# CognitiveAISystems/pogema

Hardware: AMD Instinct MI355X
Metric: agent-steps/sec (whole node), 64-agent 64x64 grid, batch=8192 envs (higher is better)
Workload: dtype u32

## Files before the change

include/pogema_amd.h:

```cpp
#ifndef POGEMA_AMD_H
#define POGEMA_AMD_H

#include <stddef.h>
#include <stdint.h>

#ifdef __cplusplus
extern "C" {
#endif

#define PGX_ABI_VERSION 6

#define PGX_OK 0
#define PGX_E_INVALID (-1)
#define PGX_E_HIP (-2)
#define PGX_E_NOMEM (-3)
#define PGX_E_STATE (-4)
#define PGX_E_PLACEMENT (-5)

#define PGX_COLLISION_PRIORITY 0
#define PGX_COLLISION_BLOCK_BOTH 1
#define PGX_COLLISION_SOFT 2

#define PGX_ON_TARGET_FINISH 0
#define PGX_ON_TARGET_RESTART 1
// ... 51 lines not shown
int pgx_abi_version(void);
const char* pgx_last_error(void);

int pgx_create(const pgx_config* cfg, int device, pgx_env** out);
int pgx_destroy(pgx_env* env);
int pgx_check_config(const pgx_config* cfg);

int64_t pgx_obs_elems(const pgx_env* env);
int64_t pgx_agent_elems(const pgx_env* env);

int pgx_reset_from_state(pgx_env* env, const uint8_t* obstacles, const int32_t* agent_xy,
                         const int32_t* target_xy, void* stream);

int pgx_reset_random(pgx_env* env, float density, uint64_t seed, const uint8_t* shared_map,
                     const uint8_t* env_mask, int32_t max_retries, void* stream);

int pgx_regenerate(pgx_env* env, const uint8_t* env_mask, float density, uint64_t seed, const uint8_t* shared_map,
                   int32_t max_retries, void* obs, void* stream);
int64_t pgx_regenerate_failures(pgx_env* env, void* stream);

int pgx_set_map_pool(pgx_env* env, const uint8_t* maps, int32_t num_maps, int32_t* capacity_out, void* stream);
int pgx_reset_pool(pgx_env* env, uint64_t seed, const uint8_t* env_mask, int32_t max_retries, void* stream);
int pgx_regenerate_pool(pgx_env* env, const uint8_t* env_mask, uint64_t seed, int32_t max_retries, void* obs,
                        void* stream);
int pgx_get_map_index(pgx_env* env, int32_t* map_index, void* stream);

int pgx_get_map(pgx_env* env, uint8_t* obstacles, void* stream);

int pgx_step(pgx_env* env, const void* actions, int action_dtype, void* obs, float* rewards,
             uint8_t* terminated, uint8_t* truncated, uint8_t* is_active, void* stream);

int pgx_step_held(pgx_env* env, const void* actions, int action_dtype, void* obs, uint8_t* held, int32_t refresh,
                  float* rewards, uint8_t* terminated, uint8_t* truncated, uint8_t* is_active, void* stream);
int pgx_held_available(const pgx_env* env);

int pgx_xcd_shares(pgx_env* env, int32_t* shares);
int pgx_xcd_tune(pgx_env* env, void* obs, void* obs_alt, int32_t rounds, float* us_equal, float* us_tuned, void* stream);

typedef struct pgx_geometry {
    int32_t lanes_per_env;
    int32_t waves;
    int32_t envs_per_wave;
    int32_t multi_wave;
    int32_t p16;
    int32_t stagger;
    int32_t store_policy;
    int32_t state_stores;
    int32_t grid;
    int32_t lds_bytes;
    int32_t for_rollout;
    int32_t xcd_aware;
} pgx_geometry;
int pgx_get_geometry(const pgx_env* env, int32_t for_rollout, pgx_geometry* out);

typedef struct pgx_rollout_io {
    const void* actions;
    void* obs;
    float* rewards;
    uint8_t* terminated;
    uint8_t* truncated;
    uint8_t* is_active;
    uint8_t* episode_done;
    float* metrics;
    int32_t action_dtype;
    int32_t obs_slots;
    int64_t obs_slot_stride;
// ... 141 lines not shown
```

pogema_amd/_lib.py:

```python
from __future__ import annotations

import ctypes as C
import os

_HERE = os.path.dirname(os.path.abspath(__file__))
LIB_PATH = os.environ.get("PGX_LIB") or os.path.join(_HERE, "libpogema_amd.so")

PGX_ABI_VERSION = 6

COLLISION_SYSTEMS = {"priority": 0, "block_both": 1, "soft": 2}
ON_TARGET = {"finish": 0, "restart": 1, "nothing": 2}
ACTION_DTYPES = {"int8": 0, "int32": 1, "int64": 2}
SOFT_VERTEX_RULES = {"lowest_index": 0, "all_stay": 1}
SOFT_OCCUPANCY = {"index_order": 0, "exact": 1}
COOP_REWARDS = {"all_solved": 0, "per_agent": 1}
BAD_ACTIONS = {"noop": 0, "flag": 1}
LIFELONG_RNGS = {"build": 0, "numpy": 1}
def _obs_dtypes():
    import torch
    return {torch.float32: 0, torch.uint8: 1, torch.bfloat16: 2, torch.float16: 3}


def obs_elem_bytes(dtype) -> int:
    import torch
# ... 9 lines not shown
    def __contains__(self, k):
        self._fill()
        return dict.__contains__(self, k)

    def __getitem__(self, k):
        self._fill()
        return dict.__getitem__(self, k)


OBS_DTYPES = _LazyObsDtypes()
METRIC_NAMES = ("ISR", "CSR", "ep_length", "SoC", "makespan", "avg_throughput")
MAX_OBS_RADIUS, MAX_AGENTS, MAX_SIDE = 15, 1024, 1024
MAX_NEIGHBOURS = 32
DIRECTIONS_FORMATS = {"float32": 0, "uint8": 1, "bits": 2}
SHIELD_TIE_BREAKS = {None: 0, "distance": 1}
MAX_PLAN_HORIZON = 256
PLAN_FIXED_PRIORITY = 1
OUTCOMES = ("STAY", "MOVED", "OBSTACLE", "SWAP", "OCCUPIED", "FOLLOW", "CONTESTED")
NUM_OUTCOMES = len(OUTCOMES)
POLICY_CHANNELS = {"obstacles": 0, "agents": 1, "target": 2, "other_goals": 3, "up": 4, "down": 5, "left": 6, "right": 7}
NUM_CHANNELS = len(POLICY_CHANNELS)
COPY_NO_CACHE = 1
DEFAULT_POLICY_CHANNELS = ("obstacles", "agents", "target", "up", "down", "left", "right")
GLOBAL_CHANNELS = {"obstacles": 0, "agents": 1, "targets": 2, "agent_ids": 3, "target_ids": 4}
NUM_GLOBAL_CHANNELS = len(GLOBAL_CHANNELS)
DEFAULT_GLOBAL_CHANNELS = ("obstacles", "agents", "targets")
GLOBAL_ID_CHANNELS = ("agent_ids", "target_ids")
GLOBAL_ID_MAX = {1: 255, 2: 256}
GLOBAL_BAND_CELLS = 8192


EXPORTED_SYMBOLS = (
    "pgx_abi_version", "pgx_last_error", "pgx_create", "pgx_check_config", "pgx_destroy", "pgx_obs_elems", "pgx_agent_elems",
    "pgx_reset_from_state", "pgx_reset_random", "pgx_regenerate", "pgx_regenerate_failures", "pgx_get_map", "pgx_step", "pgx_step_held", "pgx_held_available", "pgx_observe", "pgx_set_metrics_buffers", "pgx_get_state", "pgx_generate", "pgx_place_agents",
    "pgx_snapshot_bytes", "pgx_save_snapshot", "pgx_load_snapshot", "pgx_time_observe", "pgx_bad_action_count",
    "pgx_buffers_create", "pgx_buffers_ptr", "pgx_buffers_get_info", "pgx_buffers_destroy", "pgx_set_targets",
    "pgx_np_streams", "pgx_np_streams_host", "pgx_np_generate", "pgx_np_generate_host", "pgx_rollout", "pgx_buffers_stride", "pgx_buffers_drop", "pgx_xcd_shares", "pgx_xcd_tune", "pgx_buffers_create_at", "pgx_time_observe_pair", "pgx_buffers_va_reserved", "pgx_get_geometry",
    "pgx_expert_actions", "pgx_set_map_pool", "pgx_reset_pool", "pgx_regenerate_pool", "pgx_get_map_index",
    "pgx_cost_to_go", "pgx_cost_to_go_bytes", "pgx_cost_to_go_builds", "pgx_visible_agents", "pgx_pibt_actions",
    "pgx_goal_directions", "pgx_shield_actions", "pgx_pibt_plan", "pgx_move_outcomes",
    "pgx_policy_input", "pgx_copy_envs", "pgx_global_state", "pgx_global_state_check",
)


class PgxError(RuntimeError):
    def __init__(self, code: int, message: str):
        super().__init__(f"pogema_amd engine error {code}: {message}")
        self.code = code


class PgxBuffersInfo(C.Structure):
    _fields_ = [("bytes", C.c_int64), ("count", C.c_int32), ("spread", C.c_int32), ("candidates", C.c_int32),
                ("reserved0", C.c_int32), ("same_zone_us", C.c_float), ("final_us", C.c_float), ("spacer_gib", C.c_double),
                ("buffer_gbs", C.c_float), ("reserved1", C.c_float)]


class PgxGeometry(C.Structure):
    _fields_ = [(n, C.c_int32) for n in ("lanes_per_env", "waves", "envs_per_wave", "multi_wave", "p16", "stagger",
                                          "store_policy", "state_stores", "grid", "lds_bytes", "for_rollout", "xcd_aware")]


class PgxRolloutIO(C.Structure):
    _fields_ = [("actions", C.c_void_p), ("obs", C.c_void_p), ("rewards", C.c_void_p), ("terminated", C.c_void_p),
                ("truncated", C.c_void_p), ("is_active", C.c_void_p), ("episode_done", C.c_void_p), ("metrics", C.c_void_p),
                ("action_dtype", C.c_int32), ("obs_slots", C.c_int32), ("obs_slot_stride", C.c_int64),
                ("policy_seed", C.c_uint64), ("policy_step0", C.c_int64), ("actions_out", C.c_void_p)]

# ... 95 lines not shown
    lib.pgx_move_outcomes.argtypes = [vp, vp, i32, i32, vp, vp, vp, vp, vp]
    lib.pgx_move_outcomes.restype = C.c_int
    lib.pgx_policy_input.argtypes = [vp, C.POINTER(i32), i32, i32, vp, vp]
    lib.pgx_policy_input.restype = C.c_int
    lib.pgx_global_state.argtypes = [vp, C.POINTER(i32), i32, i32, vp, vp]
    lib.pgx_global_state.restype = C.c_int
    lib.pgx_global_state_check.argtypes = [i32, C.POINTER(i32), i32, i32, vp]
    lib.pgx_global_state_check.restype = C.c_int
    lib.pgx_copy_envs.argtypes = [vp, vp, vp, i32, i32, vp]
    lib.pgx_copy_envs.restype = C.c_int
    lib.pgx_set_map_pool.argtypes = [vp, vp, i32, vp, vp]
    lib.pgx_set_map_pool.restype = C.c_int
    lib.pgx_reset_pool.argtypes = [vp, u64, vp, i32, vp]
    lib.pgx_reset_pool.restype = C.c_int
    lib.pgx_regenerate_pool.argtypes = [vp, vp, u64, i32, vp, vp]
    lib.pgx_regenerate_pool.restype = C.c_int
    lib.pgx_get_map_index.argtypes = [vp, vp, vp]
    lib.pgx_get_map_index.restype = C.c_int
    lib.pgx_set_targets.argtypes = [vp, vp, vp, vp]
    lib.pgx_set_targets.restype = C.c_int
    lib.pgx_bad_action_count.argtypes = [vp, vp]
    lib.pgx_bad_action_count.restype = i64
    lib.pgx_time_observe.argtypes = [vp, vp, i32, C.POINTER(C.c_float), vp]
    lib.pgx_time_observe.restype = C.c_int
    lib.pgx_time_observe_pair.argtypes = [vp, vp, vp, i32, C.POINTER(C.c_float), vp]
    lib.pgx_time_observe_pair.restype = C.c_int
    lib.pgx_snapshot_bytes.argtypes = [vp]
    lib.pgx_snapshot_bytes.restype = i64
    lib.pgx_save_snapshot.argtypes = [vp, vp, vp]
    lib.pgx_load_snapshot.argtypes = [vp, vp, vp]
    lib.pgx_save_snapshot.restype = lib.pgx_load_snapshot.restype = C.c_int
    lib.pgx_step.argtypes = [vp, vp, C.c_int, vp, vp, vp, vp, vp, vp]
    lib.pgx_step_held.argtypes = [vp, vp, C.c_int, vp, vp, i32, vp, vp, vp, vp, vp]
    lib.pgx_held_available.argtypes = [vp]
    lib.pgx_step_held.restype = lib.pgx_held_available.restype = C.c_int
    lib.pgx_observe.argtypes = [vp, vp, vp]
    lib.pgx_set_metrics_buffers.argtypes = [vp, vp, vp]
    lib.pgx_get_state.argtypes = [vp, vp, vp, vp, vp, vp, vp]
    lib.pgx_generate.argtypes = [i32, i32, i32, i32, f32, u64, i64, i32, i32, vp, vp, vp]
    lib.pgx_place_agents.argtypes = [i32, i32, i32, i32, u64, i64, i32, i32, vp, i32, vp, vp]
    for name in ("pgx_create", "pgx_destroy", "pgx_reset_from_state", "pgx_reset_random", "pgx_regenerate", "pgx_get_map",
                 "pgx_step", "pgx_observe", "pgx_set_metrics_buffers", "pgx_set_metrics_buffers",
                 "pgx_get_state", "pgx_generate", "pgx_place_agents"):
        getattr(lib, name).restype = C.c_int
    if lib.pgx_abi_version() != PGX_ABI_VERSION:
        raise ImportError(f"{LIB_PATH}: ABI version {lib.pgx_abi_version()} != expected {PGX_ABI_VERSION}; rebuild")
    _lib = lib
    return lib


def check(status: int) -> None:
    if status != 0:
        msg = load().pgx_last_error()
        raise PgxError(status, msg.decode("utf-8", "replace") if msg else "unknown error")
```

pogema_amd/buffers.py:

```python
from __future__ import annotations

import atexit
import collections
import contextlib
import ctypes as C
import os
import threading

import numpy as np
import torch

from . import _lib

_TYPESTR = {torch.float32: "<f4", torch.uint8: "|u1", torch.float16: "<f2", torch.bfloat16: "<f2"}


class _Owner:

    def __init__(self, lib, handle):
        self._lib, self._handle = lib, handle

    def __del__(self):
        try:
            if self._handle is not None and self._handle.value:
# ... 303 lines not shown
    _HOOK = hook
    return hook


_UNSET = object()
_HOOK = _UNSET


class RecyclingOutputs:

    @staticmethod
    def available() -> bool:
        return storage_count_hook() is not None

    def __init__(self, obs_tensors, batch: int, agents: int, zone_ptrs=()):
        if not self.available():
            raise RuntimeError("torch._C._storage_Use_Count is missing or changed its meaning in this torch build")
        self._count = storage_count_hook()
        self._zone_ptrs = frozenset(int(p) for p in zone_ptrs)
        dev = obs_tensors[0].device
        n = batch * agents
        self._sets = []
        for obs in obs_tensors:
            block = torch.empty(n * 7 + 16, dtype=torch.uint8, device=dev)
            members = (obs, block[:4 * n].view(torch.float32).view(batch, agents),
                       block[4 * n:5 * n].view(torch.bool).view(batch, agents),
                       block[5 * n:6 * n].view(torch.bool).view(batch, agents),
                       block[6 * n:7 * n].view(torch.bool).view(batch, agents))
            storages = (obs.untyped_storage(), block.untyped_storage())
            self._sets.append((members, storages, tuple(st._cdata for st in storages)))
        del obs, block, members, storages
        self._idle = [tuple(self._count(c) for c in cdata) for _, _, cdata in self._sets]
        self._held = [torch.full((batch, agents), 255, dtype=torch.uint8, device=dev) for _ in self._sets]
        self._vouched = [None] * len(self._sets)
        self._next = 0
        self.taken = 0
        self.misses = 0

    def __len__(self):
        return len(self._sets)

    def obs_pointers(self):
        return [members[0].data_ptr() for members, _, _ in self._sets]

    def _is_idle(self, i: int) -> bool:
        cdata, idle = self._sets[i][2], self._idle[i]
        return self._count(cdata[0]) == idle[0] and self._count(cdata[1]) == idle[1]

    def free_sets(self) -> int:
        return sum(self._is_idle(i) for i in range(len(self._sets)))

    def retire(self):
        idle = [i for i in range(len(self._sets)) if self._is_idle(i)]
        out = [self._sets[i][0][0] for i in idle if self._sets[i][0][0].data_ptr() in self._zone_ptrs]
        for i in reversed(idle):
            del self._sets[i]
            del self._idle[i]
            del self._held[i]
            del self._vouched[i]
        self._next = 0
        return out

    def _take_index(self):
        n = len(self._sets)
        for k in range(n):
            i = (self._next + k) % n
            if self._is_idle(i):
                self._next = (i + 1) % n
                self.taken += 1
                return i
        self.misses += 1
        return None

    def _hand_out(self, i: int, with_obs: bool):
        m = self._sets[i][0]
        return (m[0].detach() if with_obs else None, m[1].detach(), m[2].detach(), m[3].detach(), m[4].detach())

    @staticmethod
    def _version(t):
        try:
            return t._version
        except Exception:
            return None

    def take(self, with_obs: bool = True):
        i = self._take_index()
        if i is None:
            return None
        if with_obs:
            self._vouched[i] = None
        return self._hand_out(i, with_obs)

    def take_for_step(self, with_obs: bool = True):
        i = self._take_index()
        if i is None:
            return None
        trusted = False
        if with_obs:
            v = self._vouched[i]
            trusted = v is not None and self._version(self._sets[i][0][0]) == v
            self._vouched[i] = None
        return self._hand_out(i, with_obs), self._held[i], trusted, i

    def vouch(self, i: int):
        self._vouched[i] = self._version(self._sets[i][0][0])
```

pogema_amd/csrc/pgx_api.cpp:

```cpp
#include "../../include/pogema_amd.h"

#include <hip/hip_runtime.h>

#include <algorithm>
#include <cstdarg>
#include <cstdio>
#include <cstdlib>
#include <cstring>
#include <new>
#include <string>
#include <vector>

#include "pgx_internal.h"

namespace {
thread_local std::string g_err;
}

namespace pgx {
int fail_msg(int code, const char* fmt, ...) {
    char buf[512];
    va_list ap;
    va_start(ap, fmt);
    vsnprintf(buf, sizeof buf, fmt, ap);
// ... 881 lines not shown
int pgx_get_map(pgx_env* e, uint8_t* obstacles, void* stream) {
    if (!e || !obstacles) return fail_msg(PGX_E_INVALID, "pgx_get_map: null argument");
    DeviceGuard guard;
    if (const int rc = enter(guard, e, "pgx_get_map", true)) return rc;
    PGX_HIP(hipMemcpyAsync(obstacles, e->map_u8, (size_t)e->cfg.batch * e->cfg.height * e->cfg.width,
                           hipMemcpyDeviceToDevice, (hipStream_t)stream));
    return PGX_OK;
}

int pgx_step(pgx_env* e, const void* actions, int action_dtype, void* obs, float* rewards, uint8_t* terminated,
             uint8_t* truncated, uint8_t* is_active, void* stream) {
    if (!e || !actions || !rewards || !terminated || !truncated) return fail_msg(PGX_E_INVALID, "pgx_step: null argument");
    if (const int rc = check_action_dtype("pgx_step", action_dtype)) return rc;
    DeviceGuard guard;
    if (const int rc = enter(guard, e, "pgx_step", true)) return rc;
    pgx::StepParams p = step_params(e, e->geo);
    p.mode = pgx::MODE_STEP;
    p.action_dtype = action_dtype;
    p.actions = actions;
    p.obs = static_cast<float*>(obs);
    p.rewards = rewards;
    p.terminated = terminated;
    p.truncated = truncated;
    p.act_out = is_active;
    PGX_HIP(pgx::launch_step(p, e->geo, (hipStream_t)stream));
    return PGX_OK;
}

int pgx_held_available(const pgx_env* e) {
    if (!e) return 0;
    return pgx::held_available(e->geo, e->cfg.num_agents, e->W, obs_elem_bytes(e->cfg.obs_dtype)) ? 1 : 0;
}

int pgx_step_held(pgx_env* e, const void* actions, int action_dtype, void* obs, uint8_t* held, int32_t refresh, float* rewards,
                  uint8_t* terminated, uint8_t* truncated, uint8_t* is_active, void* stream) {
    if (!e || !obs || !held || !pgx_held_available(e))
        return pgx_step(e, actions, action_dtype, obs, rewards, terminated, truncated, is_active, stream);
    if (!actions || !rewards || !terminated || !truncated) return fail_msg(PGX_E_INVALID, "pgx_step_held: null argument");
    if (const int rc = check_action_dtype("pgx_step_held", action_dtype)) return rc;
    DeviceGuard guard;
    if (const int rc = enter(guard, e, "pgx_step_held", true)) return rc;
    pgx::StepParams p = step_params(e, e->geo);
    p.mode = pgx::MODE_STEP;
    p.action_dtype = action_dtype;
    p.actions = actions;
    p.obs = static_cast<float*>(obs);
    p.rewards = rewards;
    p.terminated = terminated;
    p.truncated = truncated;
    p.act_out = is_active;
    PGX_HIP(pgx::launch_step_held(p, e->geo, held, refresh != 0, (hipStream_t)stream));
    return PGX_OK;
}

int pgx_rollout(pgx_env* e, int32_t steps, const pgx_rollout_io* io, void* stream) {
    if (!e || !io || !io->rewards || !io->terminated || !io->truncated)
        return fail_msg(PGX_E_INVALID, "pgx_rollout: null argument");
    if (io->policy_step0 < 0 || io->policy_step0 > ((int64_t)1 << 40))
        return fail_msg(PGX_E_INVALID, "pgx_rollout: policy_step0 outside 0..2^40");
    if (steps < 1) return fail_msg(PGX_E_INVALID, "pgx_rollout: steps must be >= 1, got %d", steps);
    if (const int rc = check_action_dtype("pgx_rollout", io->action_dtype)) return rc;
    if (io->obs && io->obs_slots < 1) return fail_msg(PGX_E_INVALID, "pgx_rollout: obs given but obs_slots = %d", io->obs_slots);
    DeviceGuard guard;
    if (const int rc = enter(guard, e, "pgx_rollout", true)) return rc;
    pgx::StepParams p = step_params(e, e->geo_roll);
    p.mode = pgx::MODE_STEP;
    p.action_dtype = io->action_dtype;
    p.actions = io->actions;
    p.obs = static_cast<float*>(io->obs);
    p.rewards = io->rewards;
    p.terminated = io->terminated;
    p.truncated = io->truncated;
    p.act_out = io->is_active;
    p.metrics_out = io->metrics;
    p.episode_done = io->episode_done;
    const int64_t agents = (int64_t)e->cfg.batch * e->cfg.num_agents;
    const int64_t W = 2 * e->cfg.obs_radius + 1;
    static const int64_t action_bytes[3] = {1, 4, 8};
    pgx::RolloutParams rp;
    rp.steps = steps;
    rp.obs_slots = io->obs ? io->obs_slots : 1;
    rp.resident_bitmap = e->geo_roll.resident_bitmap ? 1 : 0;
    rp.reserved0 = 0;
    rp.actions_stride = agents * action_bytes[io->action_dtype];
    rp.agents_stride = agents;
// ... 553 lines not shown
```

pogema_amd/csrc/pgx_internal.h:

```cpp
#pragma once
#include <hip/hip_runtime.h>
#include <stddef.h>
#include <stdint.h>

namespace pgx {

int fail_msg(int code, const char* fmt, ...);

#define PGX_HIP(call)                                                                                                      \
    do {                                                                                                                   \
        const hipError_t e__ = (call);                                                                                     \
        if (e__ != hipSuccess)                                                                                             \
            return pgx::fail_msg(PGX_E_HIP, "%s failed: %s (%s:%d)", #call, hipGetErrorString(e__), __FILE__, __LINE__); \
    } while (0)

struct DeviceGuard {
    int prev = -1;
    bool changed = false;
    hipError_t err = hipSuccess;
    DeviceGuard() = default;
    explicit DeviceGuard(int dev) { (void)select(dev); }
    DeviceGuard(const DeviceGuard&) = delete;
    DeviceGuard& operator=(const DeviceGuard&) = delete;
    hipError_t select(int dev) {
// ... 79 lines not shown
    int32_t xcd_base[8];
    uint32_t flags;
    uint64_t seed;
    int64_t env_index_base;
    const uint32_t* obst;
    uint32_t* pos;
    uint32_t* tgt;
    uint8_t* active;
    int32_t* elapsed;
    const uint32_t* pos0;
    const uint32_t* tgt0;
    const uint32_t* comp_begin;
    const uint32_t* comp_len;
    const uint32_t* comp_cells;
    uint32_t* tcount;
    NpGen* np_state;
    const NpGen* np_state0;
    int4* macc;
    float* metrics_out;
    uint8_t* episode_done;
    uint32_t* bad_count;
    const void* actions;
    float* obs;
    float* rewards;
    uint8_t* terminated;
    uint8_t* truncated;
    uint8_t* act_out;
    const uint8_t* only;
    unsigned long long* dbg;
};

struct HeldParams {
    uint8_t* held;
    int32_t refresh;
    int32_t lds_word;
    int32_t words;
};

struct RolloutParams {
    int32_t steps;
    int32_t obs_slots;
    int32_t resident_bitmap;
    int32_t reserved0;
    int64_t actions_stride;
    int64_t agents_stride;
    int64_t envs_stride;
    int64_t obs_stride;
    uint64_t policy_seed;
    int64_t policy_step0;
    int8_t* actions_out;
};

struct StepGeometry {
    int G;
    int waves;
    int epw;
    bool multi_wave;
    bool p16;
    int stagger;
    int store_policy;
    int state_stores;
    bool big;
    bool pc;
    bool resident_bitmap;
    size_t lds_bytes;
    int grid;
    int32_t xcd_n[8], xcd_base[8];
};
StepGeometry step_geometry(int batch, int A, int bmw, int W, bool allow_p16, int epw_override, int obs_elem_bytes,
                           int waves_override, bool for_rollout = false);
hipError_t prepare_step(const StepGeometry& g, const StepGeometry& roll);
hipError_t raise_lds_limit(const void* fn, size_t lds_bytes);
hipError_t launch_step(const StepParams& p, const StepGeometry& g, hipStream_t stream);
bool held_available(const StepGeometry& g, int A, int W, int obs_elem_bytes);
hipError_t prepare_step_held(const StepGeometry& g, int A, int W);
hipError_t launch_step_held(const StepParams& p, const StepGeometry& g, uint8_t* held, bool refresh, hipStream_t stream);
int xcd_partition(int blocks, const float w[8], int32_t n[8], int32_t base[8]);
hipError_t launch_rollout(const StepParams& p, const RolloutParams& rp, const StepGeometry& g, hipStream_t stream);

hipError_t launch_pack_obstacles(const uint8_t* obstacles, const uint8_t* only, uint32_t* bm, int batch, int H, int Wd,
                                 int r, int wpr, int bmw, const OutsideParams& outside, hipStream_t stream);

struct ResetParams {
    int32_t env_begin, env_count;
    int32_t H, Wd, A, r, wpr, bmw;
    int32_t lifelong;
    int32_t given_state;
    int32_t max_retries;
    uint32_t thr;
    uint64_t gen_seed;
    int64_t env_index_base;
    const uint8_t* shared_map;
    uint8_t* todo;
    const uint32_t* epoch;
    uint8_t* scratch_map;
    uint32_t* labels;
    uint32_t* pending;
    uint8_t* map_u8;
    uint32_t* obst_bm;
    uint32_t *pos, *tgt, *pos0, *tgt0;
    uint8_t* active;
    uint32_t* tcount;
    NpGen* np_state;
    const NpGen* np_state0;
    int32_t* elapsed;
    int4* macc;
    uint32_t *comp_begin, *comp_len, *comp_cells;
    uint32_t* fail_count;
    OutsideParams outside;
// ... 175 lines not shown
```

pogema_amd/csrc/pgx_kernels.hip:

```cpp
#include <hip/hip_runtime.h>
#include <stdint.h>
#include <stdlib.h>

#include <array>
#include <type_traits>
#include <map>
#include <mutex>
#include <string>
#include <vector>
#include <utility>

#include "pgx_internal.h"
#include "pgx_nprng.h"

namespace pgx {

__device__ __forceinline__ uint32_t lifelong_draw(uint64_t seed, uint64_t env_index, uint32_t agent,
                                                  uint32_t counter, uint32_t n) {
    uint64_t h = gen_sm64(seed);
    h = gen_sm64(h ^ env_index);
    h = gen_sm64(h ^ (((uint64_t)agent << 32) | counter));
    return (uint32_t)(((h >> 32) * (uint64_t)n) >> 32);
}

// ... 756 lines not shown
      }
    }
    if (dbg && tid == 0) p.dbg[(size_t)blk * 4 + (dbg2 ? 3 : 1)] = wall_clock64();
    if (!p.obs) {
        if (late_stores) emit_state(pos, tgt, active, elapsed, macc, so);
        return;
    }
    if constexpr (PC) {
        if (!do_stream) return;
    }
    if constexpr (HELD) {
        for (int i = tid; i < hp.words; i += NT) smem[hp.lds_word + i] = 0u;
    }
    lds_sync<MW>();
    if (when_stores == 1) emit_state(pos, tgt, active, elapsed, macc, so);
    int out_slot = slot;
    if constexpr (PC) out_slot = slot == 0 ? rp.obs_slots - 1 : slot - 1;
    float* const obs_out = ROLL ? reinterpret_cast<float*>(reinterpret_cast<char*>(p.obs) + (size_t)out_slot * (size_t)rp.obs_stride) : p.obs;

    if constexpr (P16) {
        const int W_rt = W, r_rt = r;
        uint32_t* rows_base = smem;
        if constexpr (ROLL) rows_base = rp.resident_bitmap ? s_occ : smem;
        if constexpr (PC) rows_base = s_obst + epw * bmw + 2 * (epw * bmw + 2 * AS);
        auto p16_phases = [&](auto wt_tag) {
        constexpr int WT = decltype(wt_tag)::value;
        const int W = WT ? WT : W_rt;
        const int r = WT ? (WT - 1) / 2 : r_rt;
        const uint32_t wmask = (1u << W) - 1u;
        constexpr int RW = WT ? (WT + 1) / 2 : 8;
        [[maybe_unused]] uint32_t held_was = 255u;
        if constexpr (HELD) {
            if (tid < nag && !hp.refresh) held_was = hp.held[(size_t)env0 * A + tid];
        }
        uint32_t rp[3][RW];
#pragma unroll
        for (int t = 0; t < 3; ++t) {
#pragma unroll
            for (int m = 0; m < RW; ++m) rp[t][m] = 0u;
            const int item = tid + t * NT;
            if (item < nag * 3) {
                const int la = item / 3;
                const int c = item - la * 3;
                const int el = MW ? 0 : (p.a_magic ? (int)__umulhi((uint32_t)la, p.a_magic) : la);
                const uint32_t cell = s_apos[la];
                const int x = (int)(cell >> 16), y = (int)(cell & 0xFFFFu);
                if (c < 2) {
                    const uint32_t* bm;
                    if constexpr (BIG) bm = c == 0 ? p.obst + (size_t)env0 * bmw : s_occ;
                    else bm = (c == 0 ? s_obst : s_occ) + el * bmw;
                    const int start = y - r;
                    const int w0 = start >> 5, sh = start & 31;
                    if constexpr (WT == 0) {
#pragma unroll
                        for (int wy = 0; wy < 16; ++wy) {
                            if (wy < W) {
                                const uint32_t* rowp = bm + (x - r + wy) * wpr + w0;
                                const uint32_t bits = (uint32_t)((((uint64_t)rowp[1] << 32) | rowp[0]) >> sh) & wmask;
                                rp[t][wy >> 1] |= bits << (16 * (wy & 1));
                            }
                        }
                    } else {
                    const uint32_t* row0 = bm + (x - r) * wpr + w0;
                        constexpr int RB = WT == 11 ? 6 : WT == 15 ? 5 : 7;
    #pragma unroll
                        for (int w8 = 0; w8 < (WT ? WT : 16); w8 += RB) {
// ... 16 lines not shown
                            }
                            asm volatile("" ::: "memory");
                        }
                    }
                } else {
                    const uint32_t tc = s_atgt[la];
                    int dx = x - (int)(tc >> 16), dy = y - (int)(tc & 0xFFFFu);
                    dx = max(-r, min(r, dx));
                    dy = max(-r, min(r, dy));
                    const int hit = r - dx;
                    const uint32_t val = (1u << (r - dy)) << (16 * (hit & 1));
#pragma unroll
                    for (int m = 0; m < RW; ++m) rp[t][m] = (m == (hit >> 1)) ? val : 0u;
                }
            }
        }
        if constexpr (HELD) {
            if (tid < nag) {
                const int la = tid;
                const uint32_t cell = s_apos[la], tc = s_atgt[la];
                const int dx = max(-r, min(r, (int)(cell >> 16) - (int)(tc >> 16)));
                const int dy = max(-r, min(r, (int)(cell & 0xFFFFu) - (int)(tc & 0xFFFFu)));
                const uint32_t now = (uint32_t)((r - dx) * W + (r - dy));
                hp.held[(size_t)env0 * A + la] = (uint8_t)now;
                if (held_was < (uint32_t)(W * W)) {
                    constexpr int UL = PGX_HELD_UNIT_LOG2;
                    const uintptr_t slice = reinterpret_cast<uintptr_t>(obs_out + (size_t)env0 * A * 3 * W * W);
                    const uintptr_t plane = slice + (size_t)(la * 3 + 2) * (size_t)(W * W) * 4;
                    const uintptr_t ub = slice >> UL;
                    const int u1 = (int)(((plane + (size_t)(W * W) * 4) >> UL) - ub);
                    const int uw = (int)(((plane + held_was * 4) >> UL) - ub), un = (int)(((plane + now * 4) >> UL) - ub);
                    for (int u = (int)(((plane + ((1u << UL) - 1u)) >> UL) - ub); u < u1; ++u)
                        if (u != uw && u != un) atomicOr(&smem[hp.lds_word + (u >> 5)], 1u << (u & 31));
                }
            }
        }
        lds_sync<MW>();
        uint16_t* rows16 = reinterpret_cast<uint16_t*>(rows_base);
#pragma unroll
        for (int t = 0; t < 3; ++t) {
            const int item = tid + t * NT;
            if (item < nag * 3) {
#pragma unroll
                for (int wy = 0; wy < (WT ? WT : 16); ++wy)
                    if (WT || wy < W) rows16[item * W + wy] = (uint16_t)(rp[t][wy >> 1] >> (16 * (wy & 1)));
            }
        }
        if (tid < 4) rows16[nag * 3 * W + tid] = 0;
        lds_sync<MW>();

        const int n = nag * 3 * W * W;
        const size_t base = (size_t)env0 * A * 3 * W * W;
        if constexpr (WT == 0) {
        if (p.obs_one && W >= 7) {
            uint16_t* o = reinterpret_cast<uint16_t*>(obs_out) + base;
            const int head = min(n, (int)((8 - (base & 7)) & 7));
            const int nvec = (n - head) >> 3;
            const int tail0 = head + (nvec << 3);
            if (tid < 16) {
                const int e = (tid < 8) ? tid : tail0 + (tid - 8);
                if ((tid < 8) ? (tid < head) : (e < n)) {
                    const int row = (int)__umulhi((uint32_t)e, p.w_magic);
                    o[e] = (uint16_t)((((uint32_t)rows16[row] >> (e - row * W)) & 1u) * p.obs_one);
                }
            }
            const bool span = MW && !(p.flags & 512u);
            const int part = (nvec + nw - 1) / nw;
            const int q0 = span ? wave * part + lane : tid, q1 = span ? min(nvec, (wave + 1) * part) : nvec;
            const int e0 = head + (q0 << 3);
            const int row0 = (int)__umulhi((uint32_t)e0, p.w_magic);
            f32x4_t* out4 = reinterpret_cast<f32x4_t*>(o + head);
            const uint32_t* rows32 = reinterpret_cast<const uint32_t*>(rows16);
            const int qs = span ? 64 : NT;
            if (q0 < q1) {
                if (p.store_policy == 0) stream_rows16_loop_h16<0>(out4, rows32, W, row0, e0 - row0 * W, q0, q1, qs, p.obs_one);
                else if (p.store_policy == 1) stream_rows16_loop_h16<1>(out4, rows32, W, row0, e0 - row0 * W, q0, q1, qs, p.obs_one);
                else stream_rows16_loop_h16<2>(out4, rows32, W, row0, e0 - row0 * W, q0, q1, qs, p.obs_one);
            }
            if (when_stores == 2) emit_state(pos, tgt, active, elapsed, macc, so);
            return;
        }
        if (p.obs_one) {
// ... 492 lines not shown
        given = upto;
        if (n[x] > grid) grid = n[x];
    }
    return grid * 8;
}

static const void* held_fn_for(const StepGeometry& g) {
    if (g.big || !g.p16) return nullptr;
    if (g.multi_wave) return reinterpret_cast<const void*>(&step_held<64, true>);
#define PGX_CASE(gg) case gg: return reinterpret_cast<const void*>(&step_held<gg, false>);
    switch (g.G) {
        PGX_CASE(1) PGX_CASE(2) PGX_CASE(4) PGX_CASE(8) PGX_CASE(16) PGX_CASE(32) PGX_CASE(64)
        default: return nullptr;
    }
#undef PGX_CASE
}

static int held_words(size_t slice_bytes) {
    const size_t units = (slice_bytes >> PGX_HELD_UNIT_LOG2) + 2;
    return (int)(units / 32 + 1);
}

bool held_available(const StepGeometry& g, int A, int W, int obs_elem_bytes) {
    if (!held_fn_for(g) || obs_elem_bytes != 4 || W > 15) return false;
    const size_t slice = (size_t)g.epw * A * 3 * W * W * 4;
    return g.lds_bytes + (size_t)held_words(slice) * 4 <= 160 * 1024;
}

hipError_t prepare_step_held(const StepGeometry& g, int A, int W) {
    const size_t slice = (size_t)g.epw * A * 3 * W * W * 4;
    return raise_lds_limit(held_fn_for(g), g.lds_bytes + (size_t)held_words(slice) * 4);
}

hipError_t launch_step_held(const StepParams& p, const StepGeometry& g, uint8_t* held, bool refresh, hipStream_t stream) {
    const void* fn = held_fn_for(g);
    if (!fn) return hipErrorInvalidValue;
    StepParams args = p;
    HeldParams h;
    const int W = 2 * p.r + 1;
    h.held = held;
    h.refresh = refresh ? 1 : 0;
    h.lds_word = (int32_t)(g.lds_bytes / 4);
    h.words = held_words((size_t)g.epw * p.num_agents * 3 * W * W * 4);
    void* kargs[] = {&args, &h};
    return hipLaunchKernel(fn, dim3(g.grid), dim3(64 * g.waves), kargs, g.lds_bytes + (size_t)h.words * 4, stream);
}

hipError_t launch_step(const StepParams& p, const StepGeometry& g, hipStream_t stream) {
    const void* fn = step_fn_for(g);
    if (!fn) return hipErrorInvalidValue;
    StepParams args = p;
    void* kargs[] = {&args};
    return hipLaunchKernel(fn, dim3(g.grid), dim3(64 * g.waves), kargs, g.lds_bytes, stream);
}


hipError_t launch_pack_obstacles(const uint8_t* obstacles, const uint8_t* only, uint32_t* bm, int batch, int H, int Wd,
                                 int r, int wpr, int bmw, const OutsideParams& outside, hipStream_t stream) {
    const size_t total = (size_t)batch * bmw;
    const int bs = 256;
    hipLaunchKernelGGL(pack_obstacles_kernel, dim3((unsigned)((total + bs - 1) / bs)), dim3(bs), 0, stream,
                       obstacles, only, bm, batch, H, Wd, r, wpr, bmw, outside);
    return hipGetLastError();
}

hipError_t launch_pack_agents(const int32_t* agent_xy, const int32_t* target_xy, uint32_t* pos, uint32_t* tgt,
                              uint32_t* pos0, uint32_t* tgt0, uint8_t* active, uint32_t* tcount, size_t n,
                              int r, hipStream_t stream, NpGen* np_state, const NpGen* np_state0) {
    const int bs = 256;
    hipLaunchKernelGGL(pack_agents_kernel, dim3((unsigned)((n + bs - 1) / bs)), dim3(bs), 0, stream, agent_xy,
                       target_xy, pos, tgt, pos0, tgt0, active, tcount, n, r, np_state, np_state0);
    return hipGetLastError();
}
// ... 37 lines not shown
```

pogema_amd/vec_env.py:

```python
from __future__ import annotations

import ctypes as C
import os
import warnings
from typing import Optional

import numpy as np
import torch

from . import _lib
from .grid_config import GridConfig
from .placement import PlacementMixin, choose_buffers
from .queries import QueryMixin
from .semantics import Semantics


def _as_device_index(device) -> int:
    dev = torch.device(device)
    if dev.type != "cuda":
        raise ValueError(f"VecPogema runs on a HIP device only, got {device!r}")
    return dev.index if dev.index is not None else torch.cuda.current_device()


def parse_map_pool(maps) -> torch.Tensor:
# ... 561 lines not shown
        if actions.dtype not in (torch.int8, torch.int32, torch.int64):
            actions = actions.to(torch.int64)
        if actions.numel() != self.batch * self.num_agents:
            raise ValueError(f"expected {self.batch}x{self.num_agents} actions, got shape {tuple(actions.shape)}")
        return actions.contiguous()

    _ACTION_CODE = {torch.int8: 0, torch.int32: 1, torch.int64: 2}

    def _check_out(self, out):
        if len(out) != 5:
            raise ValueError("out must be (obs, rewards, terminated, truncated, is_active)")
        B, A = self.batch, self.num_agents
        want = ((self.obs_shape, self.obs_dtype), ((B, A), torch.float32), ((B, A), torch.bool), ((B, A), torch.bool),
                ((B, A), torch.bool))
        for name, t, (shape, dtype) in zip(("obs", "rewards", "terminated", "truncated", "is_active"), out, want):
            if t is None and name == "obs":
                continue
            ok_dtype = t.dtype == dtype or (dtype == torch.bool and t.dtype == torch.uint8)
            if tuple(t.shape) != tuple(shape) or not ok_dtype or not t.is_contiguous() or t.device != self.device:
                raise ValueError(f"out[{name}] must be a contiguous {dtype} tensor of shape {tuple(shape)} on {self.device}")
        return out

    def step(self, actions, compute_obs: bool = True, out=None):
        actions = self._prepare_actions(actions)
        if out is not None:
            obs, rewards, terminated, truncated, is_active = self._check_out(out)
            if compute_obs and obs is None:
                raise ValueError("out[obs] is None but compute_obs=True")
        else:
            held = self._held_outputs(compute_obs) if self._held_on else None
            if held is not None:
                (obs, rewards, terminated, truncated, is_active), record, trusted, index = held
                if compute_obs:
                    _lib.check(self._lib.pgx_step_held(
                        self._handle, actions.data_ptr(), self._ACTION_CODE[actions.dtype], obs.data_ptr(), record.data_ptr(),
                        0 if trusted else 1, rewards.data_ptr(), terminated.data_ptr(), truncated.data_ptr(),
                        is_active.data_ptr(), self._stream()))
                    self._recycler.vouch(index)
                    self._held_steps += 1
                    self._held_refreshes += 0 if trusted else 1
                    infos = {"is_active": is_active, "episode_done": self.episode_done, "metrics": self.metrics}
                    if self.semantics.bad_action == "flag":
                        self._raise_on_bad_actions()
                    return self._wrap_obs(obs), rewards, terminated, truncated, infos
            elif self._held_on and self._recycler and not torch.cuda.is_current_stream_capturing():
                obs, rewards, terminated, truncated, is_active = self._alloc_outputs(compute_obs)
            else:
                obs, rewards, terminated, truncated, is_active = self._outputs(compute_obs)
        _lib.check(self._lib.pgx_step(
            self._handle, actions.data_ptr(), self._ACTION_CODE[actions.dtype],
            obs.data_ptr() if compute_obs else None, rewards.data_ptr(), terminated.data_ptr(),
            truncated.data_ptr(), is_active.data_ptr(), self._stream()))
        if self.regenerate:
            if self._reset_seed is None:
                raise RuntimeError("auto_reset='regenerate' needs reset(seed) first (random instances)")
            if self._pool is not None:
                _lib.check(self._lib.pgx_regenerate_pool(
                    self._handle, self.episode_done.data_ptr(), self._reset_seed, 3,
                    obs.data_ptr() if compute_obs else None, self._stream()))
            else:
                if self._shared is None and self.grid_config.map is not None:
                    self._shared = self._shared_map_tensor()
                _lib.check(self._lib.pgx_regenerate(
                    self._handle, self.episode_done.data_ptr(), float(self.grid_config.density), self._reset_seed,
                    self._shared.data_ptr() if self._shared is not None else None, 3,
                    obs.data_ptr() if compute_obs else None, self._stream()))
        if self.semantics.bad_action == "flag":
            self._raise_on_bad_actions()
        infos = {"is_active": is_active, "episode_done": self.episode_done, "metrics": self.metrics}
        return (self._wrap_obs(obs) if compute_obs else None), rewards, terminated, truncated, infos
# ... 157 lines not shown
```

Baseline: 5.259 billion.

## Track per-unit nonzero mask of agent plane to skip unchanged zero units in held step

Adds a per-agent byte recording which 128-byte units of the agents observation plane held nonzero data last step, and passes it through a new pgx_step_held_planes entry point. The held-step kernel computes the current nonzero mask, stores it, and marks as skippable any unit that was zero both before and now, so those stores can be elided from the obs write. This aims to cut global memory writes of the recycled observation buffer, at the cost of an extra per-agent read/write, extra LDS atomics and an extra barrier per block.

```diff
diff --git a/include/pogema_amd.h b/include/pogema_amd.h
--- a/include/pogema_amd.h
+++ b/include/pogema_amd.h
@@ -107,6 +107,9 @@
 
 int pgx_step_held(pgx_env* env, const void* actions, int action_dtype, void* obs, uint8_t* held, int32_t refresh,
                   float* rewards, uint8_t* terminated, uint8_t* truncated, uint8_t* is_active, void* stream);
+int pgx_step_held_planes(pgx_env* env, const void* actions, int action_dtype, void* obs, uint8_t* held, uint8_t* lines,
+                         int32_t refresh, float* rewards, uint8_t* terminated, uint8_t* truncated, uint8_t* is_active,
+                         void* stream);
 int pgx_held_available(const pgx_env* env);
 
 int pgx_xcd_shares(pgx_env* env, int32_t* shares);
diff --git a/pogema_amd/_lib.py b/pogema_amd/_lib.py
--- a/pogema_amd/_lib.py
+++ b/pogema_amd/_lib.py
@@ -65,7 +65,7 @@
 
 EXPORTED_SYMBOLS = (
     "pgx_abi_version", "pgx_last_error", "pgx_create", "pgx_check_config", "pgx_destroy", "pgx_obs_elems", "pgx_agent_elems",
-    "pgx_reset_from_state", "pgx_reset_random", "pgx_regenerate", "pgx_regenerate_failures", "pgx_get_map", "pgx_step", "pgx_step_held", "pgx_held_available", "pgx_observe", "pgx_set_metrics_buffers", "pgx_get_state", "pgx_generate", "pgx_place_agents",
+    "pgx_reset_from_state", "pgx_reset_random", "pgx_regenerate", "pgx_regenerate_failures", "pgx_get_map", "pgx_step", "pgx_step_held", "pgx_step_held_planes", "pgx_held_available", "pgx_observe", "pgx_set_metrics_buffers", "pgx_get_state", "pgx_generate", "pgx_place_agents",
     "pgx_snapshot_bytes", "pgx_save_snapshot", "pgx_load_snapshot", "pgx_time_observe", "pgx_bad_action_count",
     "pgx_buffers_create", "pgx_buffers_ptr", "pgx_buffers_get_info", "pgx_buffers_destroy", "pgx_set_targets",
     "pgx_np_streams", "pgx_np_streams_host", "pgx_np_generate", "pgx_np_generate_host", "pgx_rollout", "pgx_buffers_stride", "pgx_buffers_drop", "pgx_xcd_shares", "pgx_xcd_tune", "pgx_buffers_create_at", "pgx_time_observe_pair", "pgx_buffers_va_reserved", "pgx_get_geometry",
@@ -227,8 +227,9 @@
     lib.pgx_save_snapshot.restype = lib.pgx_load_snapshot.restype = C.c_int
     lib.pgx_step.argtypes = [vp, vp, C.c_int, vp, vp, vp, vp, vp, vp]
     lib.pgx_step_held.argtypes = [vp, vp, C.c_int, vp, vp, i32, vp, vp, vp, vp, vp]
+    lib.pgx_step_held_planes.argtypes = [vp, vp, C.c_int, vp, vp, vp, i32, vp, vp, vp, vp, vp]
     lib.pgx_held_available.argtypes = [vp]
-    lib.pgx_step_held.restype = lib.pgx_held_available.restype = C.c_int
+    lib.pgx_step_held.restype = lib.pgx_step_held_planes.restype = lib.pgx_held_available.restype = C.c_int
     lib.pgx_observe.argtypes = [vp, vp, vp]
     lib.pgx_set_metrics_buffers.argtypes = [vp, vp, vp]
     lib.pgx_get_state.argtypes = [vp, vp, vp, vp, vp, vp, vp]
diff --git a/pogema_amd/buffers.py b/pogema_amd/buffers.py
--- a/pogema_amd/buffers.py
+++ b/pogema_amd/buffers.py
@@ -359,6 +359,7 @@
         del obs, block, members, storages
         self._idle = [tuple(self._count(c) for c in cdata) for _, _, cdata in self._sets]
         self._held = [torch.full((batch, agents), 255, dtype=torch.uint8, device=dev) for _ in self._sets]
+        self._lines = [torch.zeros((batch, agents), dtype=torch.uint8, device=dev) for _ in self._sets]
         self._vouched = [None] * len(self._sets)
         self._next = 0
         self.taken = 0
@@ -384,6 +385,7 @@
             del self._sets[i]
             del self._idle[i]
             del self._held[i]
+            del self._lines[i]
             del self._vouched[i]
         self._next = 0
         return out
@@ -429,5 +431,8 @@
             self._vouched[i] = None
         return self._hand_out(i, with_obs), self._held[i], trusted, i
 
+    def lines(self, i: int):
+        return self._lines[i]
+
     def vouch(self, i: int):
         self._vouched[i] = self._version(self._sets[i][0][0])
diff --git a/pogema_amd/csrc/pgx_api.cpp b/pogema_amd/csrc/pgx_api.cpp
--- a/pogema_amd/csrc/pgx_api.cpp
+++ b/pogema_amd/csrc/pgx_api.cpp
@@ -937,8 +937,9 @@
     return pgx::held_available(e->geo, e->cfg.num_agents, e->W, obs_elem_bytes(e->cfg.obs_dtype)) ? 1 : 0;
 }
 
-int pgx_step_held(pgx_env* e, const void* actions, int action_dtype, void* obs, uint8_t* held, int32_t refresh, float* rewards,
-                  uint8_t* terminated, uint8_t* truncated, uint8_t* is_active, void* stream) {
+int pgx_step_held_planes(pgx_env* e, const void* actions, int action_dtype, void* obs, uint8_t* held, uint8_t* lines,
+                         int32_t refresh, float* rewards, uint8_t* terminated, uint8_t* truncated, uint8_t* is_active,
+                         void* stream) {
     if (!e || !obs || !held || !pgx_held_available(e))
         return pgx_step(e, actions, action_dtype, obs, rewards, terminated, truncated, is_active, stream);
     if (!actions || !rewards || !terminated || !truncated) return fail_msg(PGX_E_INVALID, "pgx_step_held: null argument");
@@ -954,8 +955,14 @@
     p.terminated = terminated;
     p.truncated = truncated;
     p.act_out = is_active;
-    PGX_HIP(pgx::launch_step_held(p, e->geo, held, refresh != 0, (hipStream_t)stream));
-    return PGX_OK;
+    PGX_HIP(pgx::launch_step_held(p, e->geo, held, lines, refresh != 0, (hipStream_t)stream));
+    return PGX_OK;
+}
+
+int pgx_step_held(pgx_env* e, const void* actions, int action_dtype, void* obs, uint8_t* held, int32_t refresh, float* rewards,
+                  uint8_t* terminated, uint8_t* truncated, uint8_t* is_active, void* stream) {
+    return pgx_step_held_planes(e, actions, action_dtype, obs, held, nullptr, refresh, rewards, terminated, truncated, is_active,
+                                stream);
 }
 
 int pgx_rollout(pgx_env* e, int32_t steps, const pgx_rollout_io* io, void* stream) {
diff --git a/pogema_amd/csrc/pgx_internal.h b/pogema_amd/csrc/pgx_internal.h
--- a/pogema_amd/csrc/pgx_internal.h
+++ b/pogema_amd/csrc/pgx_internal.h
@@ -135,6 +135,7 @@
 
 struct HeldParams {
     uint8_t* held;
+    uint8_t* lines;
     int32_t refresh;
     int32_t lds_word;
     int32_t words;
@@ -177,7 +178,8 @@
 hipError_t launch_step(const StepParams& p, const StepGeometry& g, hipStream_t stream);
 bool held_available(const StepGeometry& g, int A, int W, int obs_elem_bytes);
 hipError_t prepare_step_held(const StepGeometry& g, int A, int W);
-hipError_t launch_step_held(const StepParams& p, const StepGeometry& g, uint8_t* held, bool refresh, hipStream_t stream);
+hipError_t launch_step_held(const StepParams& p, const StepGeometry& g, uint8_t* held, uint8_t* lines, bool refresh,
+                            hipStream_t stream);
 int xcd_partition(int blocks, const float w[8], int32_t n[8], int32_t base[8]);
 hipError_t launch_rollout(const StepParams& p, const RolloutParams& rp, const StepGeometry& g, hipStream_t stream);
 
diff --git a/pogema_amd/csrc/pgx_kernels.hip b/pogema_amd/csrc/pgx_kernels.hip
--- a/pogema_amd/csrc/pgx_kernels.hip
+++ b/pogema_amd/csrc/pgx_kernels.hip
@@ -812,6 +812,10 @@
         [[maybe_unused]] uint32_t held_was = 255u;
         if constexpr (HELD) {
             if (tid < nag && !hp.refresh) held_was = hp.held[(size_t)env0 * A + tid];
+        }
+        [[maybe_unused]] uint32_t lines_was = 0xFFu;
+        if constexpr (HELD) {
+            if (hp.lines && tid < nag && !hp.refresh) lines_was = hp.lines[(size_t)env0 * A + tid];
         }
         uint32_t rp[3][RW];
 #pragma unroll
@@ -894,6 +898,8 @@
                     const int uw = (int)(((plane + held_was * 4) >> UL) - ub), un = (int)(((plane + now * 4) >> UL) - ub);
                     for (int u = (int)(((plane + ((1u << UL) - 1u)) >> UL) - ub); u < u1; ++u)
                         if (u != uw && u != un) atomicOr(&smem[hp.lds_word + (u >> 5)], 1u << (u & 31));
+                } else {
+                    lines_was = 0xFFu;
                 }
             }
         }
@@ -910,6 +916,36 @@
         }
         if (tid < 4) rows16[nag * 3 * W + tid] = 0;
         lds_sync<MW>();
+        if constexpr (HELD) {
+            if (hp.lines) {
+                static_assert(PGX_HELD_UNIT_LOG2 == 7, "hp.lines: one bit per 32-float unit, at most 7 per plane");
+                if (tid < nag) {
+                    const int la = tid;
+                    const uintptr_t slice = reinterpret_cast<uintptr_t>(obs_out + (size_t)env0 * A * 3 * W * W);
+                    const uintptr_t plane = slice + (size_t)(la * 3 + 1) * (size_t)(W * W) * 4;
+                    const int off = (int)(plane & 127u) >> 2;
+                    const uint16_t* mine = rows16 + (la * 3 + 1) * W;
+                    uint32_t nzj = 0u;
+#pragma unroll
+                    for (int wy = 0; wy < (WT ? WT : 16); ++wy) {
+                        if (WT || wy < W) {
+                            const int ps = off + wy * W;
+                            const uint64_t v = (uint64_t)mine[wy] << (ps & 31);
+                            nzj |= ((uint32_t)v != 0u ? 1u : 0u) << (ps >> 5);
+                            nzj |= ((uint32_t)(v >> 32) != 0u ? 1u : 0u) << ((ps >> 5) + 1);
+                        }
+                    }
+                    const int K = max(0, W * W - ((32 - off) & 31)) >> 5;
+                    const uint32_t nz = (off ? nzj >> 1 : nzj) & ((1u << K) - 1u);
+                    hp.lines[(size_t)env0 * A + la] = (uint8_t)nz;
+                    const int u0 = (int)(((plane + 127u) >> 7) - (slice >> 7));
+                    const uint64_t z = (uint64_t)(~(lines_was | nz) & ((1u << K) - 1u)) << (u0 & 31);
+                    if ((uint32_t)z) atomicOr(&smem[hp.lds_word + (u0 >> 5)], (uint32_t)z);
+                    if ((uint32_t)(z >> 32)) atomicOr(&smem[hp.lds_word + (u0 >> 5) + 1], (uint32_t)(z >> 32));
+                }
+                lds_sync<MW>();
+            }
+        }
 
         const int n = nag * 3 * W * W;
         const size_t base = (size_t)env0 * A * 3 * W * W;
@@ -1468,13 +1504,15 @@
     return raise_lds_limit(held_fn_for(g), g.lds_bytes + (size_t)held_words(slice) * 4);
 }
 
-hipError_t launch_step_held(const StepParams& p, const StepGeometry& g, uint8_t* held, bool refresh, hipStream_t stream) {
+hipError_t launch_step_held(const StepParams& p, const StepGeometry& g, uint8_t* held, uint8_t* lines, bool refresh,
+                            hipStream_t stream) {
     const void* fn = held_fn_for(g);
     if (!fn) return hipErrorInvalidValue;
     StepParams args = p;
     HeldParams h;
     const int W = 2 * p.r + 1;
     h.held = held;
+    h.lines = lines;
     h.refresh = refresh ? 1 : 0;
     h.lds_word = (int32_t)(g.lds_bytes / 4);
     h.words = held_words((size_t)g.epw * p.num_agents * 3 * W * W * 4);
diff --git a/pogema_amd/vec_env.py b/pogema_amd/vec_env.py
--- a/pogema_amd/vec_env.py
+++ b/pogema_amd/vec_env.py
@@ -617,10 +617,10 @@
             if held is not None:
                 (obs, rewards, terminated, truncated, is_active), record, trusted, index = held
                 if compute_obs:
-                    _lib.check(self._lib.pgx_step_held(
+                    _lib.check(self._lib.pgx_step_held_planes(
                         self._handle, actions.data_ptr(), self._ACTION_CODE[actions.dtype], obs.data_ptr(), record.data_ptr(),
-                        0 if trusted else 1, rewards.data_ptr(), terminated.data_ptr(), truncated.data_ptr(),
-                        is_active.data_ptr(), self._stream()))
+                        self._recycler.lines(index).data_ptr(), 0 if trusted else 1, rewards.data_ptr(), terminated.data_ptr(),
+                        truncated.data_ptr(), is_active.data_ptr(), self._stream()))
                     self._recycler.vouch(index)
                     self._held_steps += 1
                     self._held_refreshes += 0 if trusted else 1
```

New measurement: 5.300 billion (median of 2 runs). About the same (+0.8%).
